# albfre/ipm-zoo

Measured on AMD Instinct MI355X. Metric: Newton steps/sec + factor TFLOP/s, dense QP n=8192, 1/2/4/8 MI355X, higher is better.
Workload: dtype f64; 1 GPU; c3; n=8192, m=2048, p=1024, kkt_N=11264, formulation=SlackedSlacks ineq + Regularization eq (delta=1e-4), augmented LDL^T, parallelism=replicas x1 (independent QPs, one per GPU)

## Files before the change

ipm-zoo_amd/csrc/capi.cpp:

```cpp
#include <hip/hip_runtime.h>

#include <climits>
#include <cmath>
#include <cstdio>
#include <cstdlib>
#include <cstring>
#include <mutex>
#include <string>
#include <vector>

#include "ipmz.h"
#include "kernels.h"

using namespace ipmz;

namespace {
thread_local std::string g_last_error;

int fail(int code, const std::string& msg) {
  g_last_error = msg;
  return code;
}
#define HIP_OK(expr)                                                                                     \
  do {                                                                                                   \
// ... 140 lines not shown
  set_debug_inject_mask(mask);
  return IPMZ_OK;
}

int ipmz_ctx_set_blocking(ipmz_ctx* ctx, int nbo, int nbi) {
  if (!ctx) return fail(IPMZ_ERR_INVALID, "null ctx");
  if ((nbi != 64 && nbi != 128) || (nbo != 0 && (nbo < nbi || nbo % nbi != 0 || nbo > IPMZ_NBO_MAX)))
    return fail(IPMZ_ERR_INVALID, "blocking: nbi in {64,128}, nbo 0 (auto) or a multiple of nbi, <= 512");
  ctx->nbo = nbo;
  ctx->nbi = nbi;
  return IPMZ_OK;
}

int ipmz_ctx_get_blocking(ipmz_ctx* ctx, int N, int* nbo, int* nbi) {
  if (!ctx || N < 0 || !nbo || !nbi) return fail(IPMZ_ERR_INVALID, "ipmz_ctx_get_blocking: bad arguments");
  *nbo = nbo_for(ctx, N);
  *nbi = ctx->nbi;
  return IPMZ_OK;
}

namespace {
struct WsLayout {
  int64_t info_off, pctrl_off, side_off, linv_off, w_off, y_off, z_off, ctrl_off, prep_off, total;
};
WsLayout ws_layout(int N, int nbo, int nbi) {
  WsLayout l;
  const int64_t nblk = (N + nbi - 1) / nbi;
  l.info_off = 0;
  l.pctrl_off = 256;
  l.side_off = l.pctrl_off + round_up(panel_ctrl_words(N, nbo) * 4, 256);
  l.linv_off = l.side_off + round_up(2 * nbi * 8, 256);
  l.w_off = l.linv_off + round_up(nblk * nbi * nbi * 8, 256);
  l.y_off = l.w_off + round_up(3 * (int64_t)N * nbo * 8, 256);
  l.z_off = l.y_off + round_up((int64_t)N * 8, 256);
  l.ctrl_off = l.z_off + round_up((int64_t)N * 8, 256);
  l.prep_off = l.ctrl_off + 256;
  l.total = l.prep_off + (nbi == 64 ? round_up(solve_prep_elems(N) * 8, 256) : 0);
  return l;
}
hipError_t solve_ws(const double* K, int64_t ld, int N, const double* D, const char* ws, int nbo, int nbi, double* b,
                    hipStream_t st) {
  const WsLayout l = ws_layout(N, nbo, nbi);
  char* w = const_cast<char*>(ws);
  const double* Linv = reinterpret_cast<const double*>(w + l.linv_off);
  if (nbi == 64)
    return ldlt_solve_persistent(K, ld, N, D, reinterpret_cast<const double*>(w + l.prep_off), b,
                                 reinterpret_cast<double*>(w + l.y_off), reinterpret_cast<double*>(w + l.z_off),
                                 reinterpret_cast<unsigned*>(w + l.ctrl_off), st);
  return ldlt_solve(K, ld, N, D, Linv, nbi, b, reinterpret_cast<double*>(w + l.side_off), st);
}
const unsigned* panel_err_word(const char* ws, const WsLayout& l) {
  return reinterpret_cast<const unsigned*>(ws + l.pctrl_off) + PANEL_ERR_WORD;
}
const unsigned* solve_err_word(const char* ws, const WsLayout& l) {
  return reinterpret_cast<const unsigned*>(ws + l.ctrl_off) + SOLVE_ERR_WORD;
}
int ws_status(hipStream_t st, const char* ws, int N, int nbo, int nbi, const char* what) {
  const WsLayout l = ws_layout(N, nbo, nbi);
  return err_words_status(st, panel_err_word(ws, l), solve_err_word(ws, l), what);
}
int err_words_status(hipStream_t st, const unsigned* pe_word, const unsigned* se_word, const char* what) {
  unsigned pe = 0, se = 0;
  HIP_OK(hipMemcpyAsync(&pe, pe_word, 4, hipMemcpyDeviceToHost, st));
  HIP_OK(hipMemcpyAsync(&se, se_word, 4, hipMemcpyDeviceToHost, st));
  HIP_OK(hipStreamSynchronize(st));
  if (pe) return fail(IPMZ_ERR_HIP, std::string(what) + ": a hand-off inside the outer-panel factor kernel timed out "
                                                        "(spin limit 0.5 s); the factor is invalid");
  if (se) return fail(IPMZ_ERR_HIP, std::string(what) + ": a hand-off inside the persistent triangular solve timed out "
                                                        "(spin limit 0.5 s); the solution is invalid");
  return IPMZ_OK;
}
}

}

namespace {
struct BkWs {
  double *Linv = nullptr, *P = nullptr, *y = nullptr, *x = nullptr;
  unsigned* ctrl = nullptr;
  char* meta = nullptr;
  int64_t total = 0;
};
BkWs bk_ws(char* base, int N) {
  BkWs w;
  int64_t off = 0;
  auto take = [&](int64_t bytes) {
    char* p = base ? base + off : nullptr;
    off += round_up(bytes, 256);
    return p;
  };
  w.Linv = reinterpret_cast<double*>(take((int64_t)((N + 63) / 64) * 64 * 64 * 8));
  w.P = reinterpret_cast<double*>(take(solve_prep_elems(N) * 8));
  w.y = reinterpret_cast<double*>(take((int64_t)N * 8));
  w.x = reinterpret_cast<double*>(take((int64_t)N * 8));
  w.ctrl = reinterpret_cast<unsigned*>(take(256));
  w.meta = take((int64_t)bk_fast_meta_bytes(N));
  w.total = off;
  return w;
}
hipError_t bk_setup(const double* F, int64_t ld, int N, const int* ipiv, const int* info, double* LT, double* Lp,
                    int64_t ldp, const BkWs& w, hipStream_t st) {
  hipError_t e = bk_fast_prepare(F, ld, N, ipiv, info, LT, Lp, ldp, w.meta, st);
  if (e == hipSuccess) e = linv_from_l(Lp, ldp, N, 64, w.Linv, st);
  if (e == hipSuccess) e = solve_prep(Lp, ldp, N, w.Linv, w.P, st);
  if (e == hipSuccess) e = solve_reset(w.y, w.x, sizeof(double), N, w.ctrl, st);
  return e;
}
hipError_t bk_run(const double* Lp, int64_t ldp, int N, const double* LT, const int* ipiv, const BkWs& w, double* b,
                  hipStream_t st) {
  const unsigned* flag = bk_fast_flag(w.meta);
  double* t = bk_fast_tmp(w.meta, N);
  const double* ones = bk_fast_ones(w.meta, N);
  hipError_t e = bk_fast_gather(b, N, w.meta, st);
  if (e == hipSuccess) e = ldlt_solve_persistent_sweep(Lp, ldp, N, ones, w.P, t, w.y, w.x, w.ctrl, false, st, flag);
  if (e == hipSuccess) e = bk_fast_dsolve(w.y, N, w.meta, st);
  if (e == hipSuccess) e = ldlt_solve_persistent_sweep(Lp, ldp, N, ones, w.P, t, w.y, w.x, w.ctrl, true, st, flag);
  if (e == hipSuccess) e = bk_fast_scatter(b, N, w.meta, st);
  if (e == hipSuccess) e = bk_fast_fallback(LT, N, ipiv, b, w.meta, st);
  return e;
}
}

extern "C" {

int64_t ipmz_ldlt_workspace_bytes(ipmz_ctx* ctx, int N) {
  if (!ctx || N < 0) return 0;
  return ws_layout(N, nbo_for(ctx, N), ctx->nbi).total;
// ... 1486 lines not shown
```

ipm-zoo_amd/csrc/kernels.h:

```cpp
#pragma once
#include <hip/hip_runtime.h>
#include <stdint.h>
#include <stdio.h>

#define IPMZ_NBO_MAX 512
#define IPMZ_PANEL_CTRL_WORDS 320
#define IPMZ_EARLY_CHAIN_MAX_N 4096
#define IPMZ_TCHUNK 32
#define IPMZ_CHAIN_STAMP_BLOCKS 512
#define IPMZ_SOLVE_BLOCK 128
#define IPMZ_SOLVE_CTRL_WORDS 8

namespace ipmz {

enum { IPMZ_INJECT_SOLVE = 1, IPMZ_INJECT_PANEL = 2, IPMZ_INJECT_GRAPH_FORKS = 4, IPMZ_DEBUG_CONVERT_ONLY = 16,
       IPMZ_DEBUG_ONE_STREAM = 32, IPMZ_DEBUG_TRACE = 64, IPMZ_DEBUG_F32_ENGINE = 128,
       IPMZ_DEBUG_NO_FOURTH = 256, IPMZ_DEBUG_IR_FULL = 512,
       IPMZ_DEBUG_F64_ENGINE = 1024, IPMZ_DEBUG_GIVEBACK = 2048, IPMZ_DEBUG_ROWS_CHAIN = 4096,
       IPMZ_DEBUG_NO_K0 = 8192, IPMZ_DEBUG_NO_FUSED_SOLVES = 16384, IPMZ_DEBUG_READY_LATE = 32768,
       IPMZ_DEBUG_MULTI_BLOCKED = 65536, IPMZ_DEBUG_MULTI_W512 = 131072,
       IPMZ_DEBUG_MULTI_W128 = 262144 };
#define IPMZ_TRACE(...)                                                  \
  do {                                                                   \
    if (::ipmz::debug_inject_mask() & ::ipmz::IPMZ_DEBUG_TRACE) {        \
      fprintf(stderr, "[ipmz] " __VA_ARGS__);                            \
      fputc('\n', stderr);                                              \
      fflush(stderr);                                                    \
    }                                                                    \
  } while (0)
int debug_inject_mask();
hipError_t stream_record(hipEvent_t e, hipStream_t s);
hipError_t stream_wait(hipStream_t s, hipEvent_t e);
void set_capture_origin(hipStream_t s);
void set_debug_inject_mask(int mask);
constexpr int PANEL_ERR_WORD = 2;
constexpr int SOLVE_ERR_WORD = 1;

struct BatchStrides {
  int B = 1;
  int64_t sK = 0, sD = 0, sL = 0, sW = 0;
  unsigned* pflags = nullptr;
  const double* K0 = nullptr;
  int small_kernel = 0;
};
#define IPMZ_PAIR_FLAGS 32
bool small_pair_eligible(int B, int N);
bool small_pair_used(int kern, bool have_flags, int B, int N);
#define IPMZ_SMALL_NMAX 1024
hipError_t ldlt_factor_small_batched(double* K, int64_t ld, int N, double* D, double* Linv, double* W, int* info,
                                     hipStream_t st, const BatchStrides& bs);
hipError_t ldlt_factor_small_variant(int snw, double* K, int64_t ld, int N, double* D, double* Linv, double* W,
                                     int* info, hipStream_t st, const BatchStrides& bs);
hipError_t ldlt_factor_batched(double* K, int64_t ld, int N, double* D, double* Linv, double* W, int nbo, int nbi,
                               int* info, hipStream_t st, const BatchStrides& bs);
// ... 11 lines not shown
                       hipStream_t st, TrailTimer* timer, hipStream_t st2, hipStream_t st3, hipEvent_t* ev, int nev,
                       unsigned* pctrl = nullptr, hipStream_t st4 = nullptr);
#define IPMZ_PANEL_PRE00_WORDS (3 * 64 * 64 * 2)
inline int64_t panel_ctrl_words(int N, int nbo) {
  return (int64_t)IPMZ_PANEL_CTRL_WORDS * (1 + (N + nbo - 1) / nbo) + IPMZ_PANEL_PRE00_WORDS;
}
hipError_t panel_factor(double* K, int64_t ld, int N, int k0, int bo, double* D, double* Lb0, double* Wp, int ldw,
                        const double* pre00_in, double* pre00_out,
                        int* info, unsigned* area, unsigned* err, const double* Wprev, int kprev, int boprev,
                        bool rows_prev, hipStream_t st_chain, hipStream_t st_rows,
                        const unsigned* parea = nullptr, bool wait_ready = false);
hipError_t panel_factor(float* K, int64_t ld, int N, int k0, int bo, float* D, float* Lb0, float* Wp, int ldw,
                        const float* pre00_in, float* pre00_out,
                        int* info, unsigned* area, unsigned* err, const float* Wprev, int kprev, int boprev,
                        bool rows_prev, hipStream_t st_chain, hipStream_t st_rows,
                        const unsigned* parea = nullptr, bool wait_ready = false);
hipError_t panel_ready(unsigned* area, hipStream_t st);
hipError_t linv_from_l(const double* L, int64_t ld, int N, int nbi, double* Linv, hipStream_t st);
hipError_t gemm_nt_sub(int M, int N, int Kd, const double* A, int64_t lda, const double* B, int64_t ldb,
                       double* C, int64_t ldc, int64_t row0, int64_t col0, bool square_lower, hipStream_t st,
                       const BatchStrides* bs = nullptr);

hipError_t ldlt_solve(const double* K, int64_t ld, int N, const double* D, const double* Linv, int nbi, double* b,
                      double* side, hipStream_t st);

#define IPMZ_TRSM_PANEL_MAX 512
hipError_t ldlt_solve_multi(const double* K, int64_t ld, int N, const double* D, const double* Linv, int nbi,
                            double* B, int64_t ldb, int nrhs, int w, hipStream_t st);

hipError_t ldlt_solve_batched(const double* K, int64_t ld, int N, const double* D, const double* Linv, int nbi,
                              double* b, int B, int64_t sK, int64_t sD, int64_t sL, int64_t sb, hipStream_t st);

int64_t solve_prep_elems(int N);
hipError_t solve_reset(void* ybuf, void* xbuf, size_t elem, int N, unsigned* ctrl, hipStream_t st,
                       int* info = nullptr, unsigned* words = nullptr, int64_t nwords = 0, int* info2 = nullptr);
hipError_t solve_stamps(unsigned long long* out);
hipError_t chain_stamps(unsigned long long* c, unsigned long long* h);
hipError_t solve_prep(const double* K, int64_t ld, int N, const double* Linv, double* P, hipStream_t st);
hipError_t solve_prep(const float* K, int64_t ld, int N, const float* Linv, float* P, hipStream_t st);
hipError_t ldlt_solve_persistent(const double* K, int64_t ld, int N, const double* D, const double* P, double* b,
                                 double* ybuf, double* xbuf, unsigned* ctrl, hipStream_t st);
hipError_t ldlt_solve_persistent_sweep(const double* K, int64_t ld, int N, const double* D, const double* P,
                                       double* b, double* ybuf, double* xbuf, unsigned* ctrl, bool backward,
                                       hipStream_t st, const unsigned* skip);
hipError_t ldlt_solve_persistent(const float* K, int64_t ld, int N, const float* D, const float* P, float* b,
                                 float* ybuf, float* xbuf, unsigned* ctrl, hipStream_t st,
                                 const unsigned* skip = nullptr);

struct MixedWs {
  int N = 0, nbo = 256;
  int64_t ld32 = 0;
  float *K32 = nullptr, *D32 = nullptr, *Linv32 = nullptr, *W32 = nullptr, *P32 = nullptr;
  float *y32 = nullptr, *z32 = nullptr, *r32 = nullptr;
  unsigned *ctrl = nullptr, *state = nullptr, *pctrl = nullptr;
  int* info = nullptr;
  double *s = nullptr, *x = nullptr, *colp = nullptr, *rowp = nullptr, *part = nullptr;
  double* stat = nullptr;
  unsigned *hst = nullptr, *hst_dev = nullptr;
  hipEvent_t hev = nullptr;
  int last_iters = 2;
};
int64_t mixed_ws_bytes(int N, int nbo);
int64_t mixed_ws_carve(char* base, int N, int nbo, MixedWs& w);
hipError_t mixed_factor(const double* K, int64_t ld, MixedWs& w, hipStream_t st, hipStream_t st2, hipStream_t st3,
                        hipEvent_t* ev, int nev, TrailTimer* timer = nullptr, hipStream_t st4 = nullptr);
hipError_t mixed_solve(const double* K, int64_t ld, MixedWs& w, double* b, double tol, int max_refine,
// ... 103 lines not shown
```

ipm-zoo_amd/csrc/mixed.hip:

```cpp
#include <algorithm>

#include "common.h"
#include "kernels.h"

namespace ipmz {

namespace {
constexpr int MNT = 256;
enum { ST_DONE = 0, ST_ITERS = 1 };
}

__global__ void k_mx_scale(const double* __restrict__ K, int64_t ld, int N, double* __restrict__ s) {
  const int i = blockIdx.x * MNT + threadIdx.x;
  if (i < N) {
    const double d = fabs(K[(int64_t)i * ld + i]);
    s[i] = d > 0.0 ? 1.0 / sqrt(d) : 1.0;
  }
}

__global__ __launch_bounds__(MNT) void k_mx_to_f32(const double* __restrict__ K, int64_t ld, int N,
                                                   const double* __restrict__ s, float* __restrict__ K32,
                                                   int64_t ld32) {
  const int i = blockIdx.x;
  const double si = s[i];
// ... 137 lines not shown
    else state[ST_ITERS] = iters + 1u;
    if (hst) {
      hst[ST_ITERS] = iters;
      hst[ST_DONE] = ratio <= tol ? 1u : 0u;
    }
  }
}

__global__ void k_mx_finish(int N, const double* __restrict__ x, double* __restrict__ b) {
  const int i = blockIdx.x * MNT + threadIdx.x;
  if (i < N) b[i] = x[i];
}

int64_t mixed_ws_bytes(int N, int nbo) {
  MixedWs w;
  return mixed_ws_carve(nullptr, N, nbo, w);
}

int64_t mixed_ws_carve(char* base, int N, int nbo, MixedWs& w) {
  const int64_t nblk = (N + 63) / 64;
  int64_t off = 0;
  auto take = [&](int64_t bytes) {
    char* p = base ? base + off : nullptr;
    off += (bytes + 255) / 256 * 256;
    return p;
  };
  w.N = N;
  w.nbo = nbo;
  w.ld32 = (N + 63) / 64 * 64;
  w.K32 = reinterpret_cast<float*>(take((int64_t)N * w.ld32 * 4));
  w.D32 = reinterpret_cast<float*>(take((int64_t)N * 4));
  w.Linv32 = reinterpret_cast<float*>(take(nblk * 64 * 64 * 4));
  w.W32 = reinterpret_cast<float*>(take(3 * (int64_t)N * nbo * 4));
  w.y32 = reinterpret_cast<float*>(take((int64_t)N * 4));
  w.z32 = reinterpret_cast<float*>(take((int64_t)N * 4));
  w.r32 = reinterpret_cast<float*>(take((int64_t)N * 4));
  w.ctrl = reinterpret_cast<unsigned*>(take(IPMZ_SOLVE_CTRL_WORDS * 4));
  w.P32 = reinterpret_cast<float*>(take(solve_prep_elems(N) * 4));
  w.state = reinterpret_cast<unsigned*>(take(64));
  w.info = reinterpret_cast<int*>(take(64));
  w.pctrl = reinterpret_cast<unsigned*>(take(panel_ctrl_words(N, nbo) * 4));
  w.s = reinterpret_cast<double*>(take((int64_t)N * 8));
  w.x = reinterpret_cast<double*>(take((int64_t)N * 8));
  w.colp = reinterpret_cast<double*>(take(nblk * N * 8));
  w.rowp = reinterpret_cast<double*>(take((int64_t)NSPLIT * N * 8));
  w.part = reinterpret_cast<double*>(take(2 * ((N + 63) / 64) * 8));
  w.stat = reinterpret_cast<double*>(take(64));
  return off;
}

hipError_t mixed_factor(const double* K, int64_t ld, MixedWs& w, hipStream_t st, hipStream_t st2, hipStream_t st3,
                        hipEvent_t* ev,
                        int nev, TrailTimer* timer, hipStream_t st4) {
  const int N = w.N;
  if (N <= 0) return hipSuccess;
  hipLaunchKernelGGL(k_mx_scale, dim3((N + MNT - 1) / MNT), dim3(MNT), 0, st, K, ld, N, w.s);
  hipLaunchKernelGGL(k_mx_to_f32, dim3(N), dim3(MNT), 0, st, K, ld, N, w.s, w.K32, w.ld32);
  hipError_t e = solve_reset(w.y32, w.z32, sizeof(float), N, w.ctrl, st, w.info, w.pctrl,
                             panel_ctrl_words(N, w.nbo));
  if (e != hipSuccess) return e;
  if (debug_inject_mask() & IPMZ_DEBUG_CONVERT_ONLY) return hipGetLastError();
  return ldlt_factor(w.K32, w.ld32, N, w.D32, w.Linv32, w.W32, w.nbo, 64, w.info, st, timer, st2, st3, ev, nev,
                     w.pctrl, st4);
}

hipError_t mixed_solve(const double* K, int64_t ld, MixedWs& w, double* b, double tol, int max_refine,
                       hipStream_t st) {
  const int N = w.N;
// ... 40 lines not shown
```

ipm-zoo_amd/csrc/trsv_persist.hip:

```cpp
#include "common.h"
#include "kernels.h"
#include "sync.h"

namespace ipmz {

__device__ unsigned long long g_sstamp[2][256][6];
#ifdef IPMZ_SOLVE_STAMPS
#define SSTAMP(J, i) \
  if (tid == 0 && (J) < 256) g_sstamp[0][J][i] = __builtin_amdgcn_s_memrealtime()
#else
#define SSTAMP(J, i)
#endif
namespace {
constexpr int SB = IPMZ_SOLVE_BLOCK;
constexpr int SNT = 512;
constexpr int RP_ROWS = 4, RP_LANES = 16;
constexpr int CP_ROWS = 8, CP_LANES = 32;
constexpr int XS_LD = SB + 4;
constexpr int TDS = 65;
enum { SC_TICKET = 2, SC_TICKET_B = 3 };

template <typename T>
__device__ __forceinline__ bool is_sentinel(T v);
template <>
// ... 131 lines not shown
      XTo[c * SB + r] = (T)v;
    }
    return;
  }
  zero4(acc);
  zero4(bot);
  if (part <= 2) {
    T* Mo = M + (int64_t)J * SB * SB;
    put64<false>(Ls, va);
    __syncthreads();
    mm64<false>(acc, Xa, Ls);
    mm64<false>(bot, X21, Ls);
    __syncthreads();
    put64<false>(Ls, vb);
    __syncthreads();
    mm64<false>(bot, Xb, Ls);
    out4(Mo, 0, 64 * h, acc, R);
    out4(Mo, 64, 64 * h, bot, R);
  } else {
    T* Qo = Q + (int64_t)J * SB * SB;
    put64<true>(Ls, va);
    __syncthreads();
    mm64<true>(acc, Xa, Ls);
    __syncthreads();
    put64<true>(Ls, vb);
    __syncthreads();
    mm64<true>(acc, X21, Ls);
    mm64<true>(bot, Xb, Ls);
    out4(Qo, 0, 64 * h, acc, R);
    out4(Qo, 64, 64 * h, bot, R);
  }
}

template <typename T, bool BWD>
__global__ __launch_bounds__(SNT) void trsv128_kernel(const T* __restrict__ K, int64_t ld, int N,
                                                      const T* __restrict__ D, const T* __restrict__ X,
                                                      const T* __restrict__ XT, const T* __restrict__ M,
                                                      const T* __restrict__ Q, T* b, T* ybuf, T* xbuf,
                                                      unsigned* ctrl, int nb, const unsigned* __restrict__ skip,
                                                      int inject) {
  typedef typename Mfma<T>::vec2_t V2;
  typedef T Tile[RP_ROWS * 8];
  if (skip && *skip) return;
  __shared__ T vs[2][SB];
  __shared__ T red[SB / CP_ROWS][SB];
  __shared__ T vec[SB], bj[SB];
  __shared__ __attribute__((aligned(16))) T xs[SB * XS_LD];
  __shared__ unsigned sh_ticket, sh_stop, sh_nr[2];
  unsigned* err = ctrl + SOLVE_ERR_WORD;
  const int tid = threadIdx.x;
  const int rg = tid / RP_LANES, cg = tid % RP_LANES;
  if (tid == 0) sh_nr[0] = sh_nr[1] = 0u;

  const unsigned long long t_start = __builtin_amdgcn_s_memrealtime();
  auto stage = [&](const T* buf, int kb0, int nk, int dir) -> bool {
    for (unsigned it = 1;; ++it) {
      lds_sync();
      const int bsel = tid / SB, e = tid % SB;
      if (tid == 0) sh_nr[(it + 1) & 1] = 0u;
      if (bsel < nk) {
        const int kb = kb0 + dir * bsel;
        const int cnt = N - kb * SB < SB ? N - kb * SB : SB;
        const T v = e < cnt ? ld_sc1(&buf[(int64_t)kb * SB + e]) : T(0);
        if (e < cnt && is_sentinel(v)) sh_nr[it & 1] = 1u;
        vs[bsel][e] = v;
      }
      if (tid == 0)
        sh_stop = __builtin_amdgcn_s_memrealtime() - t_start > SPIN_TICKS || ((it & 31u) == 0u && ld_sc1(err) != 0u);
      lds_sync();
      if (!sh_nr[it & 1]) return true;
      if (sh_stop) {
        if (tid == 0) st_sc1(err, 1u);
        return false;
      }
      __builtin_amdgcn_s_sleep(1);
    }
  };
  auto load_rows = [&](Tile& t, const T* p) {
    const T* q = p + RP_ROWS * rg * SB + 2 * cg;
#pragma unroll
    for (int k = 0; k < RP_ROWS; ++k)
#pragma unroll
      for (int j = 0; j < 4; ++j) {
        const V2 v2 = *reinterpret_cast<const V2*>(q + k * SB + 32 * j);
        t[8 * k + 2 * j] = v2.x;
        t[8 * k + 2 * j + 1] = v2.y;
      }
  };
  auto put_xs = [&](const Tile& t) {
#pragma unroll
    for (int k = 0; k < RP_ROWS; ++k)
#pragma unroll
      for (int j = 0; j < 4; ++j)
        *reinterpret_cast<V2*>(&xs[(RP_ROWS * rg + k) * XS_LD + 2 * cg + 32 * j]) = V2{t[8 * k + 2 * j], t[8 * k + 2 * j + 1]};
  };
  auto dot_xs = [&](T (&acc)[RP_ROWS], const T* v) {
    T vv[8];
#pragma unroll
    for (int j = 0; j < 4; ++j) {
      const V2 v2 = *reinterpret_cast<const V2*>(v + 2 * cg + 32 * j);
      vv[2 * j] = v2.x;
      vv[2 * j + 1] = v2.y;
    }
#pragma unroll
    for (int k = 0; k < RP_ROWS; ++k)
#pragma unroll
      for (int j = 0; j < 4; ++j) {
        const V2 x2 = *reinterpret_cast<const V2*>(&xs[(RP_ROWS * rg + k) * XS_LD + 2 * cg + 32 * j]);
        acc[k] = fma(x2.x, vv[2 * j], acc[k]);
        acc[k] = fma(x2.y, vv[2 * j + 1], acc[k]);
      }
  };
  auto dot_rows = [&](T (&acc)[RP_ROWS], const Tile& t, const T* v) {
    T vv[8];
#pragma unroll
    for (int j = 0; j < 4; ++j) {
      const V2 v2 = *reinterpret_cast<const V2*>(v + 2 * cg + 32 * j);
      vv[2 * j] = v2.x;
      vv[2 * j + 1] = v2.y;
    }
#pragma unroll
    for (int k = 0; k < RP_ROWS; ++k)
#pragma unroll
      for (int i = 0; i < 8; ++i) acc[k] = fma(t[8 * k + i], vv[i], acc[k]);
  };

  for (;;) {
    lds_sync();
    if (tid == 0) sh_ticket = atomicAdd(&ctrl[BWD ? SC_TICKET_B : SC_TICKET], 1u);
    lds_sync();
    const int ticket = (int)sh_ticket;
    if (ticket >= nb) return;
    if (ticket == 0 && tid == 0) st_sc1(&ctrl[BWD ? SC_TICKET : SC_TICKET_B], 0u);

    if constexpr (!BWD) {
      const int J = ticket, J0 = J * SB;
      const int R = N - J0 < SB ? N - J0 : SB;
      SSTAMP(J, 0);
      if (tid < R) st_sc1(&xbuf[J0 + tid], sentinel<T>());
      const T* Lrow = K + (int64_t)J0 * ld;
      const int64_t ldr = ld;
      auto row_ok = [&](int k) { return RP_ROWS * rg + k < R; };
      T acc[RP_ROWS] = {T(0), T(0), T(0), T(0)};
      Tile ta, tb;
      load_rows(ta, X + (int64_t)J * SB * SB);
      if (tid < SB) bj[tid] = tid < R ? b[J0 + tid] : T(0);
      put_xs(ta);
      auto load_tile = [&](Tile& t, int Kb) {
#pragma unroll
        for (int k = 0; k < RP_ROWS; ++k)
#pragma unroll
          for (int j = 0; j < 4; ++j) {
            const int64_t row = row_ok(k) ? RP_ROWS * rg + k : 0;
            const V2 v2 = *reinterpret_cast<const V2*>(Lrow + row * ldr + (int64_t)Kb * SB + 2 * cg + 32 * j);
            t[8 * k + 2 * j] = v2.x;
            t[8 * k + 2 * j + 1] = v2.y;
          }
      };
      const int Kp = J - 2;
      const T* Mj = M + (int64_t)J * SB * SB;
      if (Kp > 0) {
        load_tile(ta, 0);
        if (Kp > 1) load_tile(tb, 1);
        else load_rows(tb, Mj);
      } else if (J >= 1) {
        if (J == 2) load_tile(ta, 0);
        load_rows(tb, Mj);
      }
      for (int Kc = 0; Kc < Kp; Kc += 2) {
        const bool two = Kc + 1 < Kp;
        if (!stage(ybuf, Kc, two ? 2 : 1, 1)) return;
        dot_rows(acc, ta, vs[0]);
        if (two) dot_rows(acc, tb, vs[1]);
        load_tile(ta, Kc + 2 < Kp ? Kc + 2 : J - 2);
        if (two) {
          if (Kc + 3 < Kp) load_tile(tb, Kc + 3);
          else load_rows(tb, Mj);
        }
      }
      if (J >= 2) {
        if (!stage(ybuf, J - 2, 1, 1)) return;
        dot_rows(acc, ta, vs[0]);
      }
      SSTAMP(J, 1);
#pragma unroll
      for (int k = 0; k < RP_ROWS; ++k) acc[k] = lanes16_sum(acc[k]);
      lds_sync();
      if (cg == 0) {
#pragma unroll
        for (int k = 0; k < RP_ROWS; ++k) {
          const int rr = RP_ROWS * rg + k;
          vec[rr] = bj[rr] - acc[k];
        }
      }
      lds_sync();
      T y[RP_ROWS] = {T(0), T(0), T(0), T(0)};
      dot_xs(y, vec);
      if (J > 0) {
        SSTAMP(J, 2);
        if (!stage(ybuf, J - 1, 1, 1)) return;
        SSTAMP(J, 4);
        T d[RP_ROWS] = {T(0), T(0), T(0), T(0)};
        dot_rows(d, tb, vs[0]);
#pragma unroll
        for (int k = 0; k < RP_ROWS; ++k) y[k] -= d[k];
      }
#pragma unroll
      for (int k = 0; k < RP_ROWS; ++k) {
        const T yk = lanes16_sum(y[k]);
        const int rr = RP_ROWS * rg + k;
        if (cg == 0 && rr < R && !(inject && J == 0)) st_sc1(&ybuf[J0 + rr], yk);
      }
      SSTAMP(J, 3);
    } else {
      const int J = nb - 1 - ticket, J0 = J * SB;
      const int R = N - J0 < SB ? N - J0 : SB;
      const bool last = J + 1 >= nb;
      const int crg = tid / CP_LANES, ccg = tid % CP_LANES;
      const bool ragged = N % SB != 0;
      T acc[4] = {T(0), T(0), T(0), T(0)};
      Tile ta, tb;
      load_rows(ta, XT + (int64_t)J * SB * SB);
      if (tid < SB) bj[tid] = tid < R ? ybuf[J0 + tid] / D[J0 + tid] : T(0);
      if (tid < R) st_sc1(&ybuf[J0 + tid], sentinel<T>());
      put_xs(ta);
      auto load_tile = [&](Tile& t, int Kb) {
        const int R0 = Kb * SB + CP_ROWS * crg;
        const T* p = K + (int64_t)R0 * ld + J0 + 2 * ccg;
        const bool rag = ragged && Kb == nb - 1;
#pragma unroll
        for (int k = 0; k < CP_ROWS; ++k)
#pragma unroll
          for (int j = 0; j < 2; ++j) {
            const bool in = !rag || R0 + k < N;
            const V2 v2 = in ? *reinterpret_cast<const V2*>(p + (int64_t)k * ld + 64 * j) : V2{T(0), T(0)};
            t[4 * k + 2 * j] = v2.x;
            t[4 * k + 2 * j + 1] = v2.y;
          }
      };
      auto dot_cols = [&](const Tile& t, const T* v) {
        T xv[CP_ROWS];
#pragma unroll
        for (int k = 0; k < CP_ROWS; k += 2) {
          const V2 v2 = *reinterpret_cast<const V2*>(v + CP_ROWS * crg + k);
          xv[k] = v2.x;
          xv[k + 1] = v2.y;
        }
#pragma unroll
        for (int k = 0; k < CP_ROWS; ++k)
#pragma unroll
          for (int i = 0; i < 4; ++i) acc[i] = fma(t[4 * k + i], xv[k], acc[i]);
      };
      const int Klo = J + 3;
      const T* Qj = Q + (int64_t)J * SB * SB;
      if (nb - 1 >= Klo) {
        load_tile(ta, nb - 1);
        if (nb - 2 >= Klo) load_tile(tb, nb - 2);
        else load_rows(tb, Qj);
      } else if (!last) {
        if (J + 2 <= nb - 1) load_tile(ta, J + 2);
        load_rows(tb, Qj);
      }
      for (int Kc = nb - 1; Kc >= Klo; Kc -= 2) {
        const bool two = Kc - 1 >= Klo;
        if (!stage(xbuf, Kc, two ? 2 : 1, -1)) return;
        dot_cols(ta, vs[0]);
        if (two) dot_cols(tb, vs[1]);
        load_tile(ta, Kc - 2 >= Klo ? Kc - 2 : J + 2);
        if (two) {
          if (Kc - 3 >= Klo) load_tile(tb, Kc - 3);
          else load_rows(tb, Qj);
        }
      }
      if (J + 2 <= nb - 1) {
        if (!stage(xbuf, J + 2, 1, 1)) return;
        dot_cols(ta, vs[0]);
      }
      lds_sync();
#pragma unroll
      for (int j = 0; j < 2; ++j) {
        red[crg][2 * ccg + 64 * j] = acc[2 * j];
        red[crg][2 * ccg + 64 * j + 1] = acc[2 * j + 1];
      }
      lds_sync();
      if (tid < SB) {
        T t = T(0);
#pragma unroll
        for (int k = 0; k < SB / CP_ROWS; ++k) t += red[k][tid];
        vec[tid] = bj[tid] - t;
      }
      lds_sync();
      T x[RP_ROWS] = {T(0), T(0), T(0), T(0)};
      dot_xs(x, vec);
      if (!last) {
        if (!stage(xbuf, J + 1, 1, 1)) return;
        T d[RP_ROWS] = {T(0), T(0), T(0), T(0)};
        dot_rows(d, tb, vs[0]);
#pragma unroll
        for (int k = 0; k < RP_ROWS; ++k) x[k] -= d[k];
      }
#pragma unroll
      for (int k = 0; k < RP_ROWS; ++k) {
        const T xk = lanes16_sum(x[k]);
        const int rr = RP_ROWS * rg + k;
        if (cg == 0 && rr < R) {
          st_sc1(&xbuf[J0 + rr], xk);
          b[J0 + rr] = xk;
        }
      }
    }
  }
}

int64_t solve_prep_elems(int N) {
  const int64_t nb = (N + SB - 1) / SB;
  return 4 * nb * SB * SB;
}

template <typename T>
static hipError_t solve_prep_t(const T* K, int64_t ld, int N, const T* Linv, T* P, hipStream_t st) {
  if (N <= 0) return hipSuccess;
  const int nb = (N + SB - 1) / SB;
  const int64_t q = (int64_t)nb * SB * SB;
  hipLaunchKernelGGL(solve_prep_kernel<T>, dim3(nb, 5), dim3(256), 0, st, K, ld, N, Linv, P, P + q, P + 2 * q,
                     P + 3 * q, nb);
  return hipGetLastError();
}
hipError_t solve_stamps(unsigned long long* out) {
  return hipMemcpyFromSymbol(out, HIP_SYMBOL(g_sstamp), sizeof(unsigned long long) * 2 * 256 * 6);
}
hipError_t solve_prep(const double* K, int64_t ld, int N, const double* Linv, double* P, hipStream_t st) {
  return solve_prep_t<double>(K, ld, N, Linv, P, st);
}
hipError_t solve_prep(const float* K, int64_t ld, int N, const float* Linv, float* P, hipStream_t st) {
  return solve_prep_t<float>(K, ld, N, Linv, P, st);
}

template <typename T>
static hipError_t solve_persistent_t(const T* K, int64_t ld, int N, const T* D, const T* P, T* b, T* ybuf, T* xbuf,
                                     unsigned* ctrl, hipStream_t st, const unsigned* skip) {
  if (N <= 0) return hipSuccess;
  if (ld % 2) return hipErrorInvalidValue;
  const int nb = (N + SB - 1) / SB;
  const int64_t q = (int64_t)nb * SB * SB;
  hipError_t e = hipSuccess;
  const int grid = nb < 256 ? nb : 256;
  const int inject = debug_inject_mask() & IPMZ_INJECT_SOLVE;
  hipLaunchKernelGGL((trsv128_kernel<T, false>), dim3(grid), dim3(SNT), 0, st, K, ld, N, D, P, P + q, P + 2 * q,
                     P + 3 * q, b, ybuf, xbuf, ctrl, nb, skip, inject);
  if ((e = hipGetLastError()) != hipSuccess) return e;
  hipLaunchKernelGGL((trsv128_kernel<T, true>), dim3(grid), dim3(SNT), 0, st, K, ld, N, D, P, P + q, P + 2 * q,
                     P + 3 * q, b, ybuf, xbuf, ctrl, nb, skip, inject);
  return hipGetLastError();
}

hipError_t ldlt_solve_persistent_sweep(const double* K, int64_t ld, int N, const double* D, const double* P,
                                       double* b, double* ybuf, double* xbuf, unsigned* ctrl, bool backward,
                                       hipStream_t st, const unsigned* skip) {
  if (N <= 0) return hipSuccess;
  if (ld % 2) return hipErrorInvalidValue;
  const int nb = (N + SB - 1) / SB;
  const int64_t q = (int64_t)nb * SB * SB;
  const int grid = nb < 256 ? nb : 256;
  const int inject = debug_inject_mask() & IPMZ_INJECT_SOLVE;
  if (backward)
    hipLaunchKernelGGL((trsv128_kernel<double, true>), dim3(grid), dim3(SNT), 0, st, K, ld, N, D, P, P + q, P + 2 * q,
                       P + 3 * q, b, ybuf, xbuf, ctrl, nb, skip, inject);
  else
    hipLaunchKernelGGL((trsv128_kernel<double, false>), dim3(grid), dim3(SNT), 0, st, K, ld, N, D, P, P + q,
                       P + 2 * q, P + 3 * q, b, ybuf, xbuf, ctrl, nb, skip, inject);
  return hipGetLastError();
}

namespace {
struct FillJob {
  unsigned* p[6];
  int64_t n[6];
  unsigned v[6];
};
__global__ __launch_bounds__(256) void fill_words_kernel(FillJob f) {
  const int r = blockIdx.y;
  unsigned* const p = f.p[r];
  const unsigned v = f.v[r];
  for (int64_t i = (int64_t)blockIdx.x * 256 + threadIdx.x; i < f.n[r]; i += (int64_t)gridDim.x * 256) p[i] = v;
}
}

hipError_t solve_reset(void* ybuf, void* xbuf, size_t elem, int N, unsigned* ctrl, hipStream_t st, int* info,
                       unsigned* words, int64_t nwords, int* info2) {
  FillJob f{};
  int cnt = 0;
  int64_t most = 0;
  auto add = [&](void* p, int64_t n, unsigned v) {
    if (!p || n <= 0) return;
    f.p[cnt] = static_cast<unsigned*>(p);
    f.n[cnt] = n;
    f.v[cnt++] = v;
    most = n > most ? n : most;
  };
  add(ctrl, IPMZ_SOLVE_CTRL_WORDS, 0u);
  add(ybuf, (int64_t)N * (int64_t)elem / 4, ~0u);
  add(xbuf, (int64_t)N * (int64_t)elem / 4, ~0u);
  add(info, 1, 0x7f7f7f7fu);
  add(info2, 1, 0x7f7f7f7fu);
  add(words, nwords, 0u);
  if (!cnt) return hipSuccess;
  const int64_t gx = (most + 255) / 256;
  hipLaunchKernelGGL(fill_words_kernel, dim3((unsigned)(gx < 64 ? gx : 64), cnt), dim3(256), 0, st, f);
  return hipGetLastError();
}

hipError_t ldlt_solve_persistent(const double* K, int64_t ld, int N, const double* D, const double* P, double* b,
                                 double* ybuf, double* xbuf, unsigned* ctrl, hipStream_t st) {
  return solve_persistent_t<double>(K, ld, N, D, P, b, ybuf, xbuf, ctrl, st, nullptr);
}
hipError_t ldlt_solve_persistent(const float* K, int64_t ld, int N, const float* D, const float* P, float* b,
                                 float* ybuf, float* xbuf, unsigned* ctrl, hipStream_t st, const unsigned* skip) {
  return solve_persistent_t<float>(K, ld, N, D, P, b, ybuf, xbuf, ctrl, st, skip);
}

}
```

Baseline: 77.49 steps/s.

## Split each persistent TRSV block-row into H parts across workgroups

The persistent blocked triangular solve kernel now divides each 128-row block into H sub-parts (4 for N up to 12288, otherwise 2), each handled by its own ticket and workgroup. Parts exchange their partial diagonal-block results through new sentinel-guarded side buffers (vbuf/ubuf), so the solve vectors double in size. The aim is more parallel workgroups on the latency-bound solve chain and less LDS per workgroup, so more fit per CU. The cost is extra inter-part spin-waits and global handoffs on the critical path of each block.

```diff
diff --git a/ipm-zoo_amd/csrc/capi.cpp b/ipm-zoo_amd/csrc/capi.cpp
--- a/ipm-zoo_amd/csrc/capi.cpp
+++ b/ipm-zoo_amd/csrc/capi.cpp
@@ -196,8 +196,8 @@
   l.linv_off = l.side_off + round_up(2 * nbi * 8, 256);
   l.w_off = l.linv_off + round_up(nblk * nbi * nbi * 8, 256);
   l.y_off = l.w_off + round_up(3 * (int64_t)N * nbo * 8, 256);
-  l.z_off = l.y_off + round_up((int64_t)N * 8, 256);
-  l.ctrl_off = l.z_off + round_up((int64_t)N * 8, 256);
+  l.z_off = l.y_off + round_up(solve_vec_elems(N) * 8, 256);
+  l.ctrl_off = l.z_off + round_up(solve_vec_elems(N) * 8, 256);
   l.prep_off = l.ctrl_off + 256;
   l.total = l.prep_off + (nbi == 64 ? round_up(solve_prep_elems(N) * 8, 256) : 0);
   return l;
@@ -255,8 +255,8 @@
   };
   w.Linv = reinterpret_cast<double*>(take((int64_t)((N + 63) / 64) * 64 * 64 * 8));
   w.P = reinterpret_cast<double*>(take(solve_prep_elems(N) * 8));
-  w.y = reinterpret_cast<double*>(take((int64_t)N * 8));
-  w.x = reinterpret_cast<double*>(take((int64_t)N * 8));
+  w.y = reinterpret_cast<double*>(take(solve_vec_elems(N) * 8));
+  w.x = reinterpret_cast<double*>(take(solve_vec_elems(N) * 8));
   w.ctrl = reinterpret_cast<unsigned*>(take(256));
   w.meta = take((int64_t)bk_fast_meta_bytes(N));
   w.total = off;
diff --git a/ipm-zoo_amd/csrc/kernels.h b/ipm-zoo_amd/csrc/kernels.h
--- a/ipm-zoo_amd/csrc/kernels.h
+++ b/ipm-zoo_amd/csrc/kernels.h
@@ -19,7 +19,7 @@
        IPMZ_DEBUG_F64_ENGINE = 1024, IPMZ_DEBUG_GIVEBACK = 2048, IPMZ_DEBUG_ROWS_CHAIN = 4096,
        IPMZ_DEBUG_NO_K0 = 8192, IPMZ_DEBUG_NO_FUSED_SOLVES = 16384, IPMZ_DEBUG_READY_LATE = 32768,
        IPMZ_DEBUG_MULTI_BLOCKED = 65536, IPMZ_DEBUG_MULTI_W512 = 131072,
-       IPMZ_DEBUG_MULTI_W128 = 262144 };
+       IPMZ_DEBUG_MULTI_W128 = 262144, IPMZ_DEBUG_SOLVE_H2 = 524288, IPMZ_DEBUG_SOLVE_H4 = 1048576 };
 #define IPMZ_TRACE(...)                                                  \
   do {                                                                   \
     if (::ipmz::debug_inject_mask() & ::ipmz::IPMZ_DEBUG_TRACE) {        \
@@ -97,6 +97,7 @@
                               double* b, int B, int64_t sK, int64_t sD, int64_t sL, int64_t sb, hipStream_t st);
 
 int64_t solve_prep_elems(int N);
+int64_t solve_vec_elems(int N);
 hipError_t solve_reset(void* ybuf, void* xbuf, size_t elem, int N, unsigned* ctrl, hipStream_t st,
                        int* info = nullptr, unsigned* words = nullptr, int64_t nwords = 0, int* info2 = nullptr);
 hipError_t solve_stamps(unsigned long long* out);
diff --git a/ipm-zoo_amd/csrc/mixed.hip b/ipm-zoo_amd/csrc/mixed.hip
--- a/ipm-zoo_amd/csrc/mixed.hip
+++ b/ipm-zoo_amd/csrc/mixed.hip
@@ -193,8 +193,8 @@
   w.D32 = reinterpret_cast<float*>(take((int64_t)N * 4));
   w.Linv32 = reinterpret_cast<float*>(take(nblk * 64 * 64 * 4));
   w.W32 = reinterpret_cast<float*>(take(3 * (int64_t)N * nbo * 4));
-  w.y32 = reinterpret_cast<float*>(take((int64_t)N * 4));
-  w.z32 = reinterpret_cast<float*>(take((int64_t)N * 4));
+  w.y32 = reinterpret_cast<float*>(take(solve_vec_elems(N) * 4));
+  w.z32 = reinterpret_cast<float*>(take(solve_vec_elems(N) * 4));
   w.r32 = reinterpret_cast<float*>(take((int64_t)N * 4));
   w.ctrl = reinterpret_cast<unsigned*>(take(IPMZ_SOLVE_CTRL_WORDS * 4));
   w.P32 = reinterpret_cast<float*>(take(solve_prep_elems(N) * 4));
diff --git a/ipm-zoo_amd/csrc/trsv_persist.hip b/ipm-zoo_amd/csrc/trsv_persist.hip
--- a/ipm-zoo_amd/csrc/trsv_persist.hip
+++ b/ipm-zoo_amd/csrc/trsv_persist.hip
@@ -187,7 +187,7 @@
   }
 }
 
-template <typename T, bool BWD>
+template <typename T, bool BWD, int H>
 __global__ __launch_bounds__(SNT) void trsv128_kernel(const T* __restrict__ K, int64_t ld, int N,
                                                       const T* __restrict__ D, const T* __restrict__ X,
                                                       const T* __restrict__ XT, const T* __restrict__ M,
@@ -195,30 +195,38 @@
                                                       unsigned* ctrl, int nb, const unsigned* __restrict__ skip,
                                                       int inject) {
   typedef typename Mfma<T>::vec2_t V2;
-  typedef T Tile[RP_ROWS * 8];
+  constexpr int RW = SB / H;
+  constexpr int RPR = RP_ROWS / H;
+  constexpr int CPT = 4 / H;
+  constexpr int TE = 8 * RPR;
+  static_assert(H == 1 || H == 2 || H == 4, "parts per block");
+  typedef T Tile[TE];
   if (skip && *skip) return;
   __shared__ T vs[2][SB];
-  __shared__ T red[SB / CP_ROWS][SB];
-  __shared__ T vec[SB], bj[SB];
-  __shared__ __attribute__((aligned(16))) T xs[SB * XS_LD];
+  __shared__ T red[SB / CP_ROWS][RW];
+  __shared__ T vec[SB], bj[RW];
+  __shared__ __attribute__((aligned(16))) T xs[RW * XS_LD];
   __shared__ unsigned sh_ticket, sh_stop, sh_nr[2];
   unsigned* err = ctrl + SOLVE_ERR_WORD;
+  T* const vbuf = ybuf + (int64_t)nb * SB;
+  T* const ubuf = xbuf + (int64_t)nb * SB;
   const int tid = threadIdx.x;
   const int rg = tid / RP_LANES, cg = tid % RP_LANES;
   if (tid == 0) sh_nr[0] = sh_nr[1] = 0u;
 
   const unsigned long long t_start = __builtin_amdgcn_s_memrealtime();
-  auto stage = [&](const T* buf, int kb0, int nk, int dir) -> bool {
+  auto stage2 = [&](const T* p0, int c0, int f0, T* d0, const T* p1, int c1, int f1, T* d1) -> bool {
     for (unsigned it = 1;; ++it) {
       lds_sync();
       const int bsel = tid / SB, e = tid % SB;
       if (tid == 0) sh_nr[(it + 1) & 1] = 0u;
-      if (bsel < nk) {
-        const int kb = kb0 + dir * bsel;
-        const int cnt = N - kb * SB < SB ? N - kb * SB : SB;
-        const T v = e < cnt ? ld_sc1(&buf[(int64_t)kb * SB + e]) : T(0);
+      const T* const p = bsel ? p1 : p0;
+      if (bsel < 2 && p) {
+        const int cnt = bsel ? c1 : c0, nfill = bsel ? f1 : f0;
+        T* const d = bsel ? d1 : d0;
+        const T v = e < cnt ? ld_sc1(&p[e]) : T(0);
         if (e < cnt && is_sentinel(v)) sh_nr[it & 1] = 1u;
-        vs[bsel][e] = v;
+        if (e < cnt || e < nfill) d[e] = v;
       }
       if (tid == 0)
         sh_stop = __builtin_amdgcn_s_memrealtime() - t_start > SPIN_TICKS || ((it & 31u) == 0u && ld_sc1(err) != 0u);
@@ -231,10 +239,16 @@
       __builtin_amdgcn_s_sleep(1);
     }
   };
+  auto stage = [&](const T* buf, int kb0, int nk, int dir) -> bool {
+    const int kb1 = kb0 + dir;
+    const int n0 = N - kb0 * SB < SB ? N - kb0 * SB : SB;
+    const int n1 = N - kb1 * SB < SB ? N - kb1 * SB : SB;
+    return stage2(buf + (int64_t)kb0 * SB, n0, SB, vs[0], nk > 1 ? buf + (int64_t)kb1 * SB : nullptr, n1, SB, vs[1]);
+  };
   auto load_rows = [&](Tile& t, const T* p) {
-    const T* q = p + RP_ROWS * rg * SB + 2 * cg;
-#pragma unroll
-    for (int k = 0; k < RP_ROWS; ++k)
+    const T* q = p + RPR * rg * SB + 2 * cg;
+#pragma unroll
+    for (int k = 0; k < RPR; ++k)
 #pragma unroll
       for (int j = 0; j < 4; ++j) {
         const V2 v2 = *reinterpret_cast<const V2*>(q + k * SB + 32 * j);
@@ -244,12 +258,12 @@
   };
   auto put_xs = [&](const Tile& t) {
 #pragma unroll
-    for (int k = 0; k < RP_ROWS; ++k)
+    for (int k = 0; k < RPR; ++k)
 #pragma unroll
       for (int j = 0; j < 4; ++j)
-        *reinterpret_cast<V2*>(&xs[(RP_ROWS * rg + k) * XS_LD + 2 * cg + 32 * j]) = V2{t[8 * k + 2 * j], t[8 * k + 2 * j + 1]};
+        *reinterpret_cast<V2*>(&xs[(RPR * rg + k) * XS_LD + 2 * cg + 32 * j]) = V2{t[8 * k + 2 * j], t[8 * k + 2 * j + 1]};
   };
-  auto dot_xs = [&](T (&acc)[RP_ROWS], const T* v) {
+  auto dot_xs = [&](T (&acc)[RPR], const T* v) {
     T vv[8];
 #pragma unroll
     for (int j = 0; j < 4; ++j) {
@@ -258,15 +272,15 @@
       vv[2 * j + 1] = v2.y;
     }
 #pragma unroll
-    for (int k = 0; k < RP_ROWS; ++k)
+    for (int k = 0; k < RPR; ++k)
 #pragma unroll
       for (int j = 0; j < 4; ++j) {
-        const V2 x2 = *reinterpret_cast<const V2*>(&xs[(RP_ROWS * rg + k) * XS_LD + 2 * cg + 32 * j]);
+        const V2 x2 = *reinterpret_cast<const V2*>(&xs[(RPR * rg + k) * XS_LD + 2 * cg + 32 * j]);
         acc[k] = fma(x2.x, vv[2 * j], acc[k]);
         acc[k] = fma(x2.y, vv[2 * j + 1], acc[k]);
       }
   };
-  auto dot_rows = [&](T (&acc)[RP_ROWS], const Tile& t, const T* v) {
+  auto dot_rows = [&](T (&acc)[RPR], const Tile& t, const T* v) {
     T vv[8];
 #pragma unroll
     for (int j = 0; j < 4; ++j) {
@@ -275,7 +289,7 @@
       vv[2 * j + 1] = v2.y;
     }
 #pragma unroll
-    for (int k = 0; k < RP_ROWS; ++k)
+    for (int k = 0; k < RPR; ++k)
 #pragma unroll
       for (int i = 0; i < 8; ++i) acc[k] = fma(t[8 * k + i], vv[i], acc[k]);
   };
@@ -285,35 +299,49 @@
     if (tid == 0) sh_ticket = atomicAdd(&ctrl[BWD ? SC_TICKET_B : SC_TICKET], 1u);
     lds_sync();
     const int ticket = (int)sh_ticket;
-    if (ticket >= nb) return;
+    if (ticket >= nb * H) return;
     if (ticket == 0 && tid == 0) st_sc1(&ctrl[BWD ? SC_TICKET : SC_TICKET_B], 0u);
 
     if constexpr (!BWD) {
-      const int J = ticket, J0 = J * SB;
+      const int J = ticket / H, h = ticket % H, J0 = J * SB, r0 = h * RW;
       const int R = N - J0 < SB ? N - J0 : SB;
-      SSTAMP(J, 0);
-      if (tid < R) st_sc1(&xbuf[J0 + tid], sentinel<T>());
-      const T* Lrow = K + (int64_t)J0 * ld;
+      const int Rh = R - r0 < RW ? R - r0 : RW;
+      if (Rh <= 0) continue;
+#ifdef IPMZ_SOLVE_STAMPS
+      const bool stamp = h == H - 1 || Rh < RW || R == r0 + RW;
+#define SSTAMPH(J, i) \
+  if (stamp) SSTAMP(J, i)
+#else
+#define SSTAMPH(J, i)
+#endif
+      SSTAMPH(J, 0);
+      if (tid < Rh) {
+        st_sc1(&xbuf[J0 + r0 + tid], sentinel<T>());
+        if (H > 1) st_sc1(&ubuf[J0 + r0 + tid], sentinel<T>());
+      }
+      const T* Lrow = K + (int64_t)(J0 + r0) * ld;
       const int64_t ldr = ld;
-      auto row_ok = [&](int k) { return RP_ROWS * rg + k < R; };
-      T acc[RP_ROWS] = {T(0), T(0), T(0), T(0)};
+      auto row_ok = [&](int k) { return RPR * rg + k < Rh; };
+      T acc[RPR];
+#pragma unroll
+      for (int k = 0; k < RPR; ++k) acc[k] = T(0);
       Tile ta, tb;
-      load_rows(ta, X + (int64_t)J * SB * SB);
-      if (tid < SB) bj[tid] = tid < R ? b[J0 + tid] : T(0);
+      load_rows(ta, X + (int64_t)J * SB * SB + r0 * SB);
+      if (tid < RW) bj[tid] = tid < Rh ? b[J0 + r0 + tid] : T(0);
       put_xs(ta);
       auto load_tile = [&](Tile& t, int Kb) {
-#pragma unroll
-        for (int k = 0; k < RP_ROWS; ++k)
+    #pragma unroll
+        for (int k = 0; k < RPR; ++k)
 #pragma unroll
           for (int j = 0; j < 4; ++j) {
-            const int64_t row = row_ok(k) ? RP_ROWS * rg + k : 0;
+            const int64_t row = row_ok(k) ? RPR * rg + k : 0;
             const V2 v2 = *reinterpret_cast<const V2*>(Lrow + row * ldr + (int64_t)Kb * SB + 2 * cg + 32 * j);
             t[8 * k + 2 * j] = v2.x;
             t[8 * k + 2 * j + 1] = v2.y;
           }
       };
       const int Kp = J - 2;
-      const T* Mj = M + (int64_t)J * SB * SB;
+      const T* Mj = M + (int64_t)J * SB * SB + r0 * SB;
       if (Kp > 0) {
         load_tile(ta, 0);
         if (Kp > 1) load_tile(tb, 1);
@@ -337,64 +365,94 @@
         if (!stage(ybuf, J - 2, 1, 1)) return;
         dot_rows(acc, ta, vs[0]);
       }
-      SSTAMP(J, 1);
-#pragma unroll
-      for (int k = 0; k < RP_ROWS; ++k) acc[k] = lanes16_sum(acc[k]);
+      SSTAMPH(J, 1);
+#pragma unroll
+      for (int k = 0; k < RPR; ++k) acc[k] = lanes16_sum(acc[k]);
       lds_sync();
       if (cg == 0) {
 #pragma unroll
-        for (int k = 0; k < RP_ROWS; ++k) {
-          const int rr = RP_ROWS * rg + k;
-          vec[rr] = bj[rr] - acc[k];
+        for (int k = 0; k < RPR; ++k) {
+          const int rr = RPR * rg + k;
+          const T v = bj[rr] - acc[k];
+          vec[r0 + rr] = v;
+          if (H > 1 && h < H - 1 && rr < Rh) st_sc1(&vbuf[J0 + r0 + rr], v);
         }
       }
-      lds_sync();
-      T y[RP_ROWS] = {T(0), T(0), T(0), T(0)};
+      if (H > 1 && tid < SB && tid >= r0 + RW) vec[tid] = T(0);
+      const bool both = H > 1 && h > 0 && J > 0;
+      if (H > 1 && h > 0) {
+        SSTAMPH(J, 2);
+        if (!stage2(vbuf + J0, r0, 0, vec, both ? ybuf + (int64_t)(J - 1) * SB : nullptr, SB, SB, vs[0])) return;
+        SSTAMPH(J, 5);
+      } else {
+        lds_sync();
+      }
+      T y[RPR];
+#pragma unroll
+      for (int k = 0; k < RPR; ++k) y[k] = T(0);
       dot_xs(y, vec);
       if (J > 0) {
-        SSTAMP(J, 2);
-        if (!stage(ybuf, J - 1, 1, 1)) return;
-        SSTAMP(J, 4);
-        T d[RP_ROWS] = {T(0), T(0), T(0), T(0)};
+        if (!both) {
+          SSTAMPH(J, 2);
+          if (!stage(ybuf, J - 1, 1, 1)) return;
+        }
+        SSTAMPH(J, 4);
+        T d[RPR];
+#pragma unroll
+        for (int k = 0; k < RPR; ++k) d[k] = T(0);
         dot_rows(d, tb, vs[0]);
 #pragma unroll
-        for (int k = 0; k < RP_ROWS; ++k) y[k] -= d[k];
-      }
-#pragma unroll
-      for (int k = 0; k < RP_ROWS; ++k) {
+        for (int k = 0; k < RPR; ++k) y[k] -= d[k];
+      }
+#pragma unroll
+      for (int k = 0; k < RPR; ++k) {
         const T yk = lanes16_sum(y[k]);
-        const int rr = RP_ROWS * rg + k;
-        if (cg == 0 && rr < R && !(inject && J == 0)) st_sc1(&ybuf[J0 + rr], yk);
-      }
-      SSTAMP(J, 3);
+        const int rr = RPR * rg + k;
+        if (cg == 0 && rr < Rh && !(inject && J == 0)) st_sc1(&ybuf[J0 + r0 + rr], yk);
+      }
+      SSTAMPH(J, 3);
+#undef SSTAMPH
     } else {
-      const int J = nb - 1 - ticket, J0 = J * SB;
+      const int J = nb - 1 - ticket / H, h = H - 1 - ticket % H, J0 = J * SB, c0 = h * RW;
       const int R = N - J0 < SB ? N - J0 : SB;
+      const int Rh = R - c0 < RW ? R - c0 : RW;
+      if (Rh <= 0) continue;
       const bool last = J + 1 >= nb;
       const int crg = tid / CP_LANES, ccg = tid % CP_LANES;
+      auto col = [&](int i) { return CPT == 4 ? 2 * ccg + 64 * (i >> 1) + (i & 1) : CPT == 2 ? 2 * ccg + i : ccg; };
       const bool ragged = N % SB != 0;
-      T acc[4] = {T(0), T(0), T(0), T(0)};
+      T acc[CPT];
+#pragma unroll
+      for (int i = 0; i < CPT; ++i) acc[i] = T(0);
       Tile ta, tb;
-      load_rows(ta, XT + (int64_t)J * SB * SB);
-      if (tid < SB) bj[tid] = tid < R ? ybuf[J0 + tid] / D[J0 + tid] : T(0);
-      if (tid < R) st_sc1(&ybuf[J0 + tid], sentinel<T>());
+      load_rows(ta, XT + (int64_t)J * SB * SB + c0 * SB);
+      if (tid < RW) bj[tid] = tid < Rh ? ybuf[J0 + c0 + tid] / D[J0 + c0 + tid] : T(0);
+      if (tid < Rh) {
+        st_sc1(&ybuf[J0 + c0 + tid], sentinel<T>());
+        if (H > 1) st_sc1(&vbuf[J0 + c0 + tid], sentinel<T>());
+      }
       put_xs(ta);
       auto load_tile = [&](Tile& t, int Kb) {
-        const int R0 = Kb * SB + CP_ROWS * crg;
-        const T* p = K + (int64_t)R0 * ld + J0 + 2 * ccg;
+            const int R0 = Kb * SB + CP_ROWS * crg;
+        const T* p = K + (int64_t)R0 * ld + J0 + c0 + (CPT > 1 ? 2 * ccg : ccg);
         const bool rag = ragged && Kb == nb - 1;
 #pragma unroll
-        for (int k = 0; k < CP_ROWS; ++k)
-#pragma unroll
-          for (int j = 0; j < 2; ++j) {
-            const bool in = !rag || R0 + k < N;
-            const V2 v2 = in ? *reinterpret_cast<const V2*>(p + (int64_t)k * ld + 64 * j) : V2{T(0), T(0)};
-            t[4 * k + 2 * j] = v2.x;
-            t[4 * k + 2 * j + 1] = v2.y;
+        for (int k = 0; k < CP_ROWS; ++k) {
+          const bool in = !rag || R0 + k < N;
+          if constexpr (CPT > 1) {
+#pragma unroll
+            for (int j = 0; j < CPT / 2; ++j) {
+              const V2 v2 = in ? *reinterpret_cast<const V2*>(p + (int64_t)k * ld + 64 * j) : V2{T(0), T(0)};
+              t[CPT * k + 2 * j] = v2.x;
+              t[CPT * k + 2 * j + 1] = v2.y;
+            }
+          } else {
+            t[k] = in ? p[(int64_t)k * ld] : T(0);
           }
+        }
       };
       auto dot_cols = [&](const Tile& t, const T* v) {
-        T xv[CP_ROWS];
+            T xv[CP_ROWS];
 #pragma unroll
         for (int k = 0; k < CP_ROWS; k += 2) {
           const V2 v2 = *reinterpret_cast<const V2*>(v + CP_ROWS * crg + k);
@@ -404,10 +462,10 @@
 #pragma unroll
         for (int k = 0; k < CP_ROWS; ++k)
 #pragma unroll
-          for (int i = 0; i < 4; ++i) acc[i] = fma(t[4 * k + i], xv[k], acc[i]);
+          for (int i = 0; i < CPT; ++i) acc[i] = fma(t[CPT * k + i], xv[k], acc[i]);
       };
       const int Klo = J + 3;
-      const T* Qj = Q + (int64_t)J * SB * SB;
+      const T* Qj = Q + (int64_t)J * SB * SB + c0 * SB;
       if (nb - 1 >= Klo) {
         load_tile(ta, nb - 1);
         if (nb - 2 >= Klo) load_tile(tb, nb - 2);
@@ -433,34 +491,47 @@
       }
       lds_sync();
 #pragma unroll
-      for (int j = 0; j < 2; ++j) {
-        red[crg][2 * ccg + 64 * j] = acc[2 * j];
-        red[crg][2 * ccg + 64 * j + 1] = acc[2 * j + 1];
-      }
+      for (int i = 0; i < CPT; ++i) red[crg][col(i)] = acc[i];
       lds_sync();
-      if (tid < SB) {
+      if (tid < RW) {
         T t = T(0);
 #pragma unroll
         for (int k = 0; k < SB / CP_ROWS; ++k) t += red[k][tid];
-        vec[tid] = bj[tid] - t;
-      }
-      lds_sync();
-      T x[RP_ROWS] = {T(0), T(0), T(0), T(0)};
+        const T u = bj[tid] - t;
+        vec[c0 + tid] = u;
+        if (H > 1 && h > 0 && tid < Rh) st_sc1(&ubuf[J0 + c0 + tid], u);
+      }
+      if (H > 1 && tid < c0) vec[tid] = T(0);
+      const bool both = H > 1 && h < H - 1 && !last;
+      if (H > 1 && h < H - 1) {
+        const int up = c0 + RW;
+        const int n1 = N - (J + 1) * SB < SB ? N - (J + 1) * SB : SB;
+        if (!stage2(ubuf + J0 + up, R - up, SB - up, vec + up, both ? xbuf + (int64_t)(J + 1) * SB : nullptr, n1, SB,
+                    vs[0]))
+          return;
+      } else {
+        lds_sync();
+      }
+      T x[RPR];
+#pragma unroll
+      for (int k = 0; k < RPR; ++k) x[k] = T(0);
       dot_xs(x, vec);
       if (!last) {
-        if (!stage(xbuf, J + 1, 1, 1)) return;
-        T d[RP_ROWS] = {T(0), T(0), T(0), T(0)};
+        if (!both && !stage(xbuf, J + 1, 1, 1)) return;
+        T d[RPR];
+#pragma unroll
+        for (int k = 0; k < RPR; ++k) d[k] = T(0);
         dot_rows(d, tb, vs[0]);
 #pragma unroll
-        for (int k = 0; k < RP_ROWS; ++k) x[k] -= d[k];
-      }
-#pragma unroll
-      for (int k = 0; k < RP_ROWS; ++k) {
+        for (int k = 0; k < RPR; ++k) x[k] -= d[k];
+      }
+#pragma unroll
+      for (int k = 0; k < RPR; ++k) {
         const T xk = lanes16_sum(x[k]);
-        const int rr = RP_ROWS * rg + k;
-        if (cg == 0 && rr < R) {
-          st_sc1(&xbuf[J0 + rr], xk);
-          b[J0 + rr] = xk;
+        const int rr = RPR * rg + k;
+        if (cg == 0 && rr < Rh) {
+          st_sc1(&xbuf[J0 + c0 + rr], xk);
+          b[J0 + c0 + rr] = xk;
         }
       }
     }
@@ -491,40 +562,63 @@
   return solve_prep_t<float>(K, ld, N, Linv, P, st);
 }
 
+int64_t solve_vec_elems(int N) {
+  const int64_t nb = (N + SB - 1) / SB;
+  return 2 * nb * SB;
+}
+
+template <typename T>
+static int solve_parts(int N) {
+  const int dbg = debug_inject_mask();
+  if ((dbg & IPMZ_DEBUG_SOLVE_H2) && (dbg & IPMZ_DEBUG_SOLVE_H4)) return 1;
+  if (dbg & IPMZ_DEBUG_SOLVE_H4) return 4;
+  if (dbg & IPMZ_DEBUG_SOLVE_H2) return 2;
+  if (N <= SB) return 1;
+  return N <= 12288 ? 4 : 2;
+}
+
+template <typename T, bool BWD, int H>
+static hipError_t launch_sweep(const T* K, int64_t ld, int N, const T* D, const T* P, T* b, T* ybuf, T* xbuf,
+                               unsigned* ctrl, hipStream_t st, const unsigned* skip) {
+  const int nb = (N + SB - 1) / SB;
+  const int64_t q = (int64_t)nb * SB * SB;
+  constexpr int RW = SB / H;
+  constexpr int64_t lds = (int64_t)sizeof(T) * (RW * XS_LD + (SB / CP_ROWS) * RW + 3 * SB + RW) + 64;
+  constexpr int by_threads = 2048 / SNT;
+  constexpr int per_cu = 160 * 1024 / lds < by_threads ? (int)(160 * 1024 / lds) : by_threads;
+  static_assert(per_cu >= 1, "a part's LDS fits a CU");
+  const int tickets = nb * H, cap = 256 * per_cu;
+  const int grid = tickets < cap ? tickets : cap;
+  const int inject = debug_inject_mask() & IPMZ_INJECT_SOLVE;
+  hipLaunchKernelGGL((trsv128_kernel<T, BWD, H>), dim3(grid), dim3(SNT), 0, st, K, ld, N, D, P, P + q, P + 2 * q,
+                     P + 3 * q, b, ybuf, xbuf, ctrl, nb, skip, inject);
+  return hipGetLastError();
+}
+template <typename T, bool BWD>
+static hipError_t sweep_t(const T* K, int64_t ld, int N, const T* D, const T* P, T* b, T* ybuf, T* xbuf,
+                          unsigned* ctrl, hipStream_t st, const unsigned* skip) {
+  if (N <= 0) return hipSuccess;
+  if (ld % 2) return hipErrorInvalidValue;
+  switch (solve_parts<T>(N)) {
+    case 4: return launch_sweep<T, BWD, 4>(K, ld, N, D, P, b, ybuf, xbuf, ctrl, st, skip);
+    case 2: return launch_sweep<T, BWD, 2>(K, ld, N, D, P, b, ybuf, xbuf, ctrl, st, skip);
+    default: return launch_sweep<T, BWD, 1>(K, ld, N, D, P, b, ybuf, xbuf, ctrl, st, skip);
+  }
+}
+
 template <typename T>
 static hipError_t solve_persistent_t(const T* K, int64_t ld, int N, const T* D, const T* P, T* b, T* ybuf, T* xbuf,
                                      unsigned* ctrl, hipStream_t st, const unsigned* skip) {
-  if (N <= 0) return hipSuccess;
-  if (ld % 2) return hipErrorInvalidValue;
-  const int nb = (N + SB - 1) / SB;
-  const int64_t q = (int64_t)nb * SB * SB;
-  hipError_t e = hipSuccess;
-  const int grid = nb < 256 ? nb : 256;
-  const int inject = debug_inject_mask() & IPMZ_INJECT_SOLVE;
-  hipLaunchKernelGGL((trsv128_kernel<T, false>), dim3(grid), dim3(SNT), 0, st, K, ld, N, D, P, P + q, P + 2 * q,
-                     P + 3 * q, b, ybuf, xbuf, ctrl, nb, skip, inject);
-  if ((e = hipGetLastError()) != hipSuccess) return e;
-  hipLaunchKernelGGL((trsv128_kernel<T, true>), dim3(grid), dim3(SNT), 0, st, K, ld, N, D, P, P + q, P + 2 * q,
-                     P + 3 * q, b, ybuf, xbuf, ctrl, nb, skip, inject);
-  return hipGetLastError();
+  const hipError_t e = sweep_t<T, false>(K, ld, N, D, P, b, ybuf, xbuf, ctrl, st, skip);
+  if (e != hipSuccess) return e;
+  return sweep_t<T, true>(K, ld, N, D, P, b, ybuf, xbuf, ctrl, st, skip);
 }
 
 hipError_t ldlt_solve_persistent_sweep(const double* K, int64_t ld, int N, const double* D, const double* P,
                                        double* b, double* ybuf, double* xbuf, unsigned* ctrl, bool backward,
                                        hipStream_t st, const unsigned* skip) {
-  if (N <= 0) return hipSuccess;
-  if (ld % 2) return hipErrorInvalidValue;
-  const int nb = (N + SB - 1) / SB;
-  const int64_t q = (int64_t)nb * SB * SB;
-  const int grid = nb < 256 ? nb : 256;
-  const int inject = debug_inject_mask() & IPMZ_INJECT_SOLVE;
-  if (backward)
-    hipLaunchKernelGGL((trsv128_kernel<double, true>), dim3(grid), dim3(SNT), 0, st, K, ld, N, D, P, P + q, P + 2 * q,
-                       P + 3 * q, b, ybuf, xbuf, ctrl, nb, skip, inject);
-  else
-    hipLaunchKernelGGL((trsv128_kernel<double, false>), dim3(grid), dim3(SNT), 0, st, K, ld, N, D, P, P + q,
-                       P + 2 * q, P + 3 * q, b, ybuf, xbuf, ctrl, nb, skip, inject);
-  return hipGetLastError();
+  return backward ? sweep_t<double, true>(K, ld, N, D, P, b, ybuf, xbuf, ctrl, st, skip)
+                  : sweep_t<double, false>(K, ld, N, D, P, b, ybuf, xbuf, ctrl, st, skip);
 }
 
 namespace {
@@ -554,8 +648,8 @@
     most = n > most ? n : most;
   };
   add(ctrl, IPMZ_SOLVE_CTRL_WORDS, 0u);
-  add(ybuf, (int64_t)N * (int64_t)elem / 4, ~0u);
-  add(xbuf, (int64_t)N * (int64_t)elem / 4, ~0u);
+  add(ybuf, solve_vec_elems(N) * (int64_t)elem / 4, ~0u);
+  add(xbuf, solve_vec_elems(N) * (int64_t)elem / 4, ~0u);
   add(info, 1, 0x7f7f7f7fu);
   add(info2, 1, 0x7f7f7f7fu);
   add(words, nwords, 0u);
```

Result: faster. 81.09 steps/s (median of 6 runs) (+4.6%).
